# uber/makisu

Measured on AMD Instinct MI355X. Metric: GiB/s hashed (Gear CDC + SHA-256 per chunk), higher is better.
Workload: dtype u32

## Files before the change

### makisu_amd/csrc/gear_cdc.hip

```cpp
#include "mi_common.h"

namespace mi {

typedef u32 u32x4 __attribute__((ext_vector_type(4)));

constexpr int kCopies      = kGearTableCopies;
constexpr int kFastCopies  = 32;
constexpr int kFastWG      = 512;
constexpr int kFastWaves   = kFastWG / 64;

constexpr int kWavesPerWG  = kGearWG / 64;
constexpr int kLaneRun     = kGearTile / 64;
constexpr int kPiece       = 128;
constexpr int kPieceUnits  = kPiece / 16;
constexpr int kBitmapWords = kGearTile / 32;
constexpr int kTableBytes  = 256 * 8 * kCopies;
constexpr int kFastTableBytes = 256 * 8 * kFastCopies;
constexpr int kFastListOff = kFastTableBytes;
constexpr int kFastLdsBytes = kFastListOff + kFastWaves * 64 * 4;
constexpr int kLdsListOff  = kTableBytes + kWavesPerWG * kBitmapWords * 4;
constexpr int kLdsFastOff  = kLdsListOff + kWavesPerWG * 64 * 4;
constexpr int kGearLdsBytes = kLdsFastOff + 16;
constexpr u32 kNoCand = 0xFFFFFFFFu;

__device__ __forceinline__ u32 lane_value(u32 v, int src) { return (u32)__builtin_amdgcn_readlane((int)v, src); }

struct CandPack { u32 a, b; };
__device__ __forceinline__ void cand_push(CandPack& pk, bool& ovf, u32 o) {
    const u32 ca = pk.a >> 30;
    if (ca < 3) { pk.a = ((ca + 1) << 30) | (((pk.a & 0x3FFFFFFFu) << 10) | o); return; }
    const u32 cb = pk.b >> 30;
    if (cb < 3) pk.b = ((cb + 1) << 30) | (((pk.b & 0x3FFFFFFFu) << 10) | o);
    else ovf = true;
}

__device__ __forceinline__ bool cand_compact(CandPack pk, bool ovf, u32 run0, int lane, u32* list) {
    const u32 ca = pk.a >> 30, cb = pk.b >> 30;
    const u32 cnt = ca + cb;
    const u64 b0 = __ballot(cnt & 1u), b1 = __ballot(cnt & 2u), b2 = __ballot(cnt & 4u);
    const u32 total = (u32)__popcll(b0) + 2u * (u32)__popcll(b1) + 4u * (u32)__popcll(b2);
    if (__ballot(ovf) || total > 64u) return false;
    const u64 below = (1ull << lane) - 1ull;
    const u32 first = (u32)__popcll(b0 & below) + 2u * (u32)__popcll(b1 & below) + 4u * (u32)__popcll(b2 & below);
    list[lane] = kNoCand;
#pragma unroll
    for (u32 k = 0; k < 3; ++k)
        if (k < ca) list[first + k] = run0 + ((pk.a >> (10 * (ca - 1 - k))) & 1023u);
    if (cb) {
#pragma unroll
        for (u32 k = 0; k < 3; ++k)
            if (k < cb) list[first + 3 + k] = run0 + ((pk.b >> (10 * (cb - 1 - k))) & 1023u);
    }
    return true;
}

__device__ __forceinline__ int bitmap_find_first(const u64* bm, int lo, int hi, int lane) {
    const int w_lo = lo >> 6, w_hi = hi >> 6;
    for (int w0 = w_lo; w0 <= w_hi; w0 += 64) {
        const int w = w0 + lane;
        u64 v = 0;
        if (w <= w_hi) v = bm[w];
        if (w == w_lo) v &= ~0ull << (lo & 63);
        if (w == w_hi) v &= ~0ull >> (63 - (hi & 63));
        const u64 bal = __ballot(v != 0);
        if (bal) {
            const int src = __ffsll((unsigned long long)bal) - 1;
            const u32 vlo = lane_value((u32)v, src), vhi = lane_value((u32)(v >> 32), src);
            const u64 vv = ((u64)vhi << 32) | vlo;
            return (w0 + src) * 64 + (__ffsll((unsigned long long)vv) - 1);
        }
    }
    return -1;
}

typedef __attribute__((address_space(3))) const u64 lds_cu64;
template <int kC>
__device__ __forceinline__ void roll16(u64& h, const u32x4 v, u32 lane_tab, u32 (&hh)[16]) {
    static_assert(kC == 8 || kC == 16 || kC == 32, "lookup address arithmetic: 64-, 128- or 256-byte entry stride");
    constexpr int kShift = kC == 8 ? 6 : 7;
    constexpr u32 kMask = 0xFFu << kShift;
    const u32 wv[4] = {v.x, v.y, v.z, v.w};
#pragma unroll
    for (int k = 0; k < 16; ++k) {
        const u32 w = wv[k >> 2];
        u32 addr;
        if constexpr (kC == 32) {
            addr = __builtin_amdgcn_perm(w, lane_tab, 0x0C020000u | ((4u + (u32)(k & 3)) << 8));
        } else {
            const int sh = 8 * (k & 3) - kShift;
            const u32 t = sh < 0 ? w << -sh : w >> sh;
            addr = __builtin_amdgcn_bitop3_b32(t, kMask, lane_tab, 0xEA);
        }
        h = (h << 1) + *(lds_cu64*)(size_t)addr;
        hh[k] = (u32)(h >> 32);
    }
}

template <int kC>
__device__ __forceinline__ u32 lds_lane_table(const u64* table, int lane) {
    const u32 base = (u32)(size_t)(__attribute__((address_space(3))) const u64*)table;
    if (base & (u32)(256 * 8 * kC - 1)) __builtin_trap();
    return base | ((u32)(lane % kC) * 8u);
}

__device__ __forceinline__ void load_piece(const u8* p, u32x4 (&d)[kPieceUnits]) {
#pragma unroll
    for (int i = 0; i < kPieceUnits; ++i) d[i] = *(const u32x4*)(p + 16 * i);
}

template <int kC, bool kBitmap>
__device__ __forceinline__ void hash16(u64& h, const u32x4 v, u32 tab, u32 thresh_m1, u32 run0, u32 base,
                                       u32* bitmap, CandPack& pk, bool& ovf) {
    u32 hh[16];
    roll16<kC>(h, v, tab, hh);
    u32 m = 0xFFFFFFFFu;
#pragma unroll
    for (int k = 0; k < 16; k += 2) m = min(m, min(hh[k], hh[k + 1]));
    if (m <= thresh_m1) {
#pragma unroll
        for (int k = 0; k < 16; ++k) {
            if (hh[k] <= thresh_m1) {
                const u32 pos = run0 + base + (u32)k;
                if (kBitmap) atomicOr(&bitmap[pos >> 5], 1u << (pos & 31));
                cand_push(pk, ovf, base + (u32)k);
            }
        }
    }
}

__device__ __forceinline__ void tile_first_loads(const u8* __restrict__ fptr, u64 ts, u32 tlen, int lane,
                                                 u32x4 (&cur)[kPieceUnits], u32x4 (&wq)[4]) {
    const u32 run0 = (u32)lane * kLaneRun;
    if (run0 >= tlen) return;
    const u8* p = fptr + ts + run0;
    load_piece(p, cur);
    if (ts + run0 != 0) {
#pragma unroll
        for (int i = 0; i < 4; ++i) wq[i] = *(const u32x4*)(p - 64 + 16 * i);
    }
}

template <int kC, bool kBitmap>
__device__ __forceinline__ void mark_tile_loaded(const u8* __restrict__ fptr, u64 ts, u32 tlen,
                                                 u32* bitmap, u32 tab, u32 thresh_m1, int lane,
                                                 u32x4 (&cur)[kPieceUnits], const u32x4 (&wq)[4],
                                                 CandPack& pk, bool& ovf) {
    pk.a = pk.b = 0;
    ovf = false;
    const u32 run0 = (u32)lane * kLaneRun;
    if (run0 >= tlen) return;
    const u8* p = fptr + ts + run0;
    const u32 run_len = tlen - run0 < (u32)kLaneRun ? tlen - run0 : (u32)kLaneRun;
    const int n_pieces = (int)((run_len + kPiece - 1) / kPiece);
    u64 h = 0;
    u32 hh[16];
    if (ts + run0 != 0) {
#pragma unroll
        for (int i = 0; i < 4; ++i) roll16<kC>(h, wq[i], tab, hh);
    }
    u32x4 nxt[kPieceUnits];
    for (int pc = 0; pc < n_pieces; ++pc) {
        if (pc + 1 < n_pieces) load_piece(p + (pc + 1) * kPiece, nxt);
#pragma unroll
        for (int g = 0; g < kPieceUnits; ++g)
            hash16<kC, kBitmap>(h, cur[g], tab, thresh_m1, run0, (u32)(pc * kPiece + g * 16), bitmap, pk, ovf);
#pragma unroll
        for (int i = 0; i < kPieceUnits; ++i) cur[i] = nxt[i];
    }
}

template <int kC, bool kBitmap>
__device__ __forceinline__ void mark_tile(const u8* __restrict__ fptr, u64 ts, u32 tlen,
                                          u32* bitmap, u32 tab, u32 thresh_m1, int lane,
                                          CandPack& pk, bool& ovf) {
    if (kBitmap) {
        u32x4* bz = (u32x4*)bitmap;
        const u32x4 z = {0, 0, 0, 0};
#pragma unroll
        for (int i = 0; i < kBitmapWords / 4 / 64; ++i) bz[i * 64 + lane] = z;
    }
    u32x4 cur[kPieceUnits], wq[4];
    tile_first_loads(fptr, ts, tlen, lane, cur, wq);
    mark_tile_loaded<kC, kBitmap>(fptr, ts, tlen, bitmap, tab, thresh_m1, lane, cur, wq, pk, ovf);
}

template <typename Emit>
__device__ __forceinline__ bool select_tile(const u32* bitmap, const u32* list, u64 ts, u32 tlen,
                                            const CdcParams& p, u64& last, int lane, Emit&& emit) {
    const u64 te = ts + tlen;
    const u32 cand = list ? list[lane] : kNoCand;
    for (;;) {
        u64 lo = last + p.min_size;
        if (lo < ts + 1) lo = ts + 1;
        u64 hi = last + p.max_size;
        if (hi > te) hi = te;
        if (lo <= hi) {
            int b;
            if (list) {
                const u32 lo_rel = (u32)(lo - ts - 1), hi_rel = (u32)(hi - ts - 1);
                const u64 bal = __ballot(cand >= lo_rel && cand <= hi_rel);
                b = bal ? (int)lane_value(cand, __ffsll((unsigned long long)bal) - 1) : -1;
            } else {
                b = bitmap_find_first((const u64*)bitmap, (int)(lo - ts - 1), (int)(hi - ts - 1), lane);
            }
            if (b >= 0) {
                last = ts + (u64)b + 1;
                if (emit(last)) return true;
                continue;
            }
        }
        if (last + p.max_size <= te) {
            last += p.max_size;
            if (emit(last)) return true;
            continue;
        }
        break;
    }
    return false;
}

__device__ __forceinline__ bool list_from_bitmap(const u32* bitmap, int lane, u32* list) {
    u32 cnt = 0;
#pragma unroll 4
    for (int w = 0; w < 32; ++w) cnt += (u32)__popc(bitmap[lane * 32 + w]);
    u32 incl = cnt;
#pragma unroll
    for (int d = 1; d < 64; d <<= 1) {
        const u32 y = __shfl_up(incl, d);
        if (lane >= d) incl += y;
    }
    const u32 total = lane_value(incl, 63);
    if (total > 64u) return false;
    list[lane] = kNoCand;
    u32 pos = incl - cnt;
    if (cnt) {
        for (int w = 0; w < 32; ++w) {
            u32 bits = bitmap[lane * 32 + w];
            while (bits) {
                const int b = __ffs(bits) - 1;
                bits &= bits - 1;
                list[pos++] = (u32)lane * kLaneRun + (u32)w * 32u + (u32)b;
            }
        }
    }
    return true;
}

template <int kC, int kWG = kGearWG>
__device__ __forceinline__ void load_table(u64* table, const u64* __restrict__ gear_table, int tid) {
    for (int i = tid; i < 256 * kC; i += kWG) table[i] = gear_table[i / kC];
}

typedef u64 u64x2 __attribute__((ext_vector_type(2)));
__device__ __forceinline__ void load_table_fast(u64* table, const u64* __restrict__ gear_table, int tid) {
    static_assert(kFastWG == 2 * 256 && kFastCopies == 32, "two threads per entry, sixteen copies each");
    const u64 g = gear_table[tid >> 1];
    const u64x2 gg = {g, g};
    u64x2* dst = (u64x2*)(table + (tid >> 1) * kFastCopies + (tid & 1) * (kFastCopies / 2));
#pragma unroll
    for (int i = 0; i < kFastCopies / 4; ++i) dst[i] = gg;
}

__global__ __launch_bounds__(kFastWG)
void gear_cdc_small_fast_kernel(const u8* __restrict__ data, const u64* __restrict__ file_off,
                                const u64* __restrict__ file_size, const u32* __restrict__ seg_file,
                                const u64* __restrict__ seg_slot, u32* __restrict__ ends32,
                                u32* __restrict__ seg_n, const u32* __restrict__ list, u32 n_list,
                                const u64* __restrict__ gear_table, CdcParams p,
                                u32* __restrict__ dense_list, u32* __restrict__ dense_count) {
    extern __shared__ __attribute__((aligned(16))) u8 smem[];
    u64* table = (u64*)smem;
    const int tid = threadIdx.x, lane = tid & 63;
    const int wave = __builtin_amdgcn_readfirstlane(tid >> 6);
    u32* cand_list = (u32*)(smem + kFastListOff) + wave * 64;
    const u32 li = blockIdx.x * kFastWaves + wave;
    const bool have = li < n_list;
    u32 s = 0;
    u64 size = 0, off = 0, slot = 0;
    if (have) {
        s = list[li];
        const u32 f = seg_file[s];
        size = file_size[f];
        off = file_off[f];
        slot = seg_slot[s];
    }
    u32x4 cur[kPieceUnits], wq[4];
    tile_first_loads(data + off, 0, (u32)size, lane, cur, wq);
    load_table_fast(table, gear_table, tid);
    __syncthreads();
    const u32 lane_tab = lds_lane_table<kFastCopies>(table, lane);
    if (!have) return;
    u32* ends = ends32 + slot;
    u64 last = 0;
    u32 n_out = 0;
    if (size) {
        CandPack pk;
        bool ovf;
        mark_tile_loaded<kFastCopies, false>(data + off, 0, (u32)size, nullptr, lane_tab, p.thresh_m1, lane, cur, wq, pk, ovf);
        if (!cand_compact(pk, ovf, (u32)lane * kLaneRun, lane, cand_list)) {
            if (lane == 0) dense_list[atomicAdd(dense_count, 1u)] = s;
            return;
        }
        __builtin_amdgcn_wave_barrier();
        select_tile(nullptr, cand_list, 0, (u32)size, p, last, lane,
                    [&](u64 c) { if (lane == 0) ends[n_out] = (u32)c; ++n_out; return false; });
    }
    if (lane == 0) {
        if (size > last) { ends[n_out] = (u32)size; ++n_out; }
        seg_n[s] = n_out;
    }
}

__global__ __launch_bounds__(kGearWG)
void gear_cdc_small_kernel(const u8* __restrict__ data, const u64* __restrict__ file_off,
                           const u64* __restrict__ file_size, const u32* __restrict__ seg_file,
                           const u64* __restrict__ seg_slot, u32* __restrict__ ends32,
                           u32* __restrict__ seg_n, const u32* __restrict__ list, u32 n_list,
                           const u32* __restrict__ n_list_dev,
                           const u64* __restrict__ gear_table, CdcParams p) {
    extern __shared__ __attribute__((aligned(16))) u8 smem[];
    u64* table = (u64*)smem;
    const int tid = threadIdx.x, lane = tid & 63, wave = tid >> 6;
    if (n_list_dev) {
        n_list = *n_list_dev;
        if (blockIdx.x * kWavesPerWG >= n_list) return;
    }
    u32* bitmap = (u32*)(smem + kTableBytes) + wave * kBitmapWords;
    u32* cand_list = (u32*)(smem + kLdsListOff) + wave * 64;
    load_table<kCopies>(table, gear_table, tid);
    __syncthreads();
    const u32 lane_tab = lds_lane_table<kCopies>(table, lane);
    const u32 li = blockIdx.x * kWavesPerWG + wave;
    if (li >= n_list) return;
    const u32 s = list[li];
    const u32 f = seg_file[s];
    const u64 size = file_size[f];
    u32* ends = ends32 + seg_slot[s];
    u64 last = 0;
    u32 n_out = 0;
    if (size) {
        CandPack pk;
        bool ovf;
        mark_tile<kCopies, true>(data + file_off[f], 0, (u32)size, bitmap, lane_tab, p.thresh_m1, lane,
                                 pk, ovf);
        const bool fast = cand_compact(pk, ovf, (u32)lane * kLaneRun, lane, cand_list);
        __builtin_amdgcn_wave_barrier();
        select_tile(bitmap, fast ? cand_list : nullptr, 0, (u32)size, p, last, lane,
                    [&](u64 c) { if (lane == 0) ends[n_out] = (u32)c; ++n_out; return false; });
    }
    if (lane == 0) {
        if (size > last) { ends[n_out] = (u32)size; ++n_out; }
        seg_n[s] = n_out;
    }
}


__device__ __forceinline__ u64 reselect_group(const u32* lists, const u32* bitmaps, u32 fast_mask,
                                               u64 g0, u64 size, u64 entry, const u32* __restrict__ spec,
                                               u32 spec_n, u64 spec_exit, u32* __restrict__ prefix,
                                               const CdcParams& p, int lane, GroupRec* rec, u32* seg_n_out,
                                               bool open_end) {
    u64 last = entry;
    u32 pcnt = 0, sidx = spec_n;
    u32 sbase = 0;
    u32 sreg = lane < (int)spec_n ? spec[lane] : kNoCand;
    bool synced = false;
    auto emit = [&](u64 c) -> bool {
        const u32 rel = (u32)(c - g0);
        for (;;) {
            const u64 bal = __ballot(sreg >= rel);
            if (bal) {
                const int i = __ffsll((unsigned long long)bal) - 1;
                if (lane_value(sreg, i) == rel && sbase + (u32)i < spec_n) { sidx = sbase + (u32)i; synced = true; }
                break;
            }
            if (sbase + 64u >= spec_n) break;
            sbase += 64u;
            sreg = sbase + (u32)lane < spec_n ? spec[sbase + lane] : kNoCand;
        }
        if (synced) return true;
        if (lane == 0) prefix[pcnt] = rel;
        ++pcnt;
        return false;
    };
    for (int t = 0; t < kWavesPerWG && !synced; ++t) {
        const u64 tts = g0 + (u64)t * kGearTile;
        if (tts >= size) break;
        const u32 tlen = (u32)((size - tts < (u64)kGearTile) ? (size - tts) : (u64)kGearTile);
        select_tile(bitmaps + t * kBitmapWords, (fast_mask >> t) & 1u ? lists + t * 64 : nullptr, tts, tlen,
                    p, last, lane, emit);
    }
    if (!synced && !open_end && g0 + kGroupBytes >= size && size > last) {
        if (!emit(size)) last = size;
    }
    const u64 exit = synced ? spec_exit : last;
    if (lane == 0) {
        rec->entry = entry;
        rec->pcnt = pcnt;
        rec->sidx = sidx;
        rec->final_exit = exit;
        rec->flags = (rec->flags & kGroupDense) | kGroupValid;
        *seg_n_out = pcnt + (spec_n - sidx);
    }
    return exit;
}

__global__ __launch_bounds__(kFastWG)
void gear_tile_mark_kernel(const u8* __restrict__ data, const u64* __restrict__ file_off,
                           const u64* __restrict__ file_size, const u32* __restrict__ group_file,
                           const u32* __restrict__ group_index, u32 n_groups,
                           u32* __restrict__ tile_lists, u32* __restrict__ tile_fast,
                           const u64* __restrict__ gear_table, CdcParams p) {
    extern __shared__ __attribute__((aligned(16))) u8 smem[];
    u64* table = (u64*)smem;
    const int tid = threadIdx.x, lane = tid & 63;
    const int wave = __builtin_amdgcn_readfirstlane(tid >> 6);
    u32* cl = (u32*)(smem + kFastListOff) + wave * 64;
    const u64 gw = (u64)blockIdx.x * kFastWaves + (u64)wave;
    const u32 g = (u32)(gw / kWavesPerWG);
    const bool have = g < n_groups;
    const int tw = (int)(gw % kWavesPerWG);
    const u64 t = (u64)g * kWavesPerWG + tw;
    u64 size = 0, off = 0, ts = 0;
    if (have) {
        const u32 f = group_file[g];
        size = file_size[f];
        off = file_off[f];
        ts = (u64)group_index[g] * kGroupBytes + (u64)tw * kGearTile;
    }
    const u32 tlen = ts >= size ? 0u : (u32)((size - ts < (u64)kGearTile) ? (size - ts) : (u64)kGearTile);
    u32x4 cur[kPieceUnits], wq[4];
    tile_first_loads(data + off, ts, tlen, lane, cur, wq);
    load_table_fast(table, gear_table, tid);
    __syncthreads();
    const u32 lane_tab = lds_lane_table<kFastCopies>(table, lane);
    if (!have) return;
    bool fast = true;
    if (tlen) {
        CandPack pk;
        bool ovf;
        mark_tile_loaded<kFastCopies, false>(data + off, ts, tlen, nullptr, lane_tab, p.thresh_m1, lane, cur, wq, pk, ovf);
        fast = cand_compact(pk, ovf, (u32)lane * kLaneRun, lane, cl);
        __builtin_amdgcn_wave_barrier();
        tile_lists[t * 64 + lane] = fast ? cl[lane] : kNoCand;
    }
    if (lane == 0) tile_fast[t] = fast ? 1u : 0u;
}

__global__ __launch_bounds__(kGearWG)
void gear_group_spec_kernel(const u64* __restrict__ file_size, const u64* __restrict__ file_seg0,
                            const u64* __restrict__ seg_slot, u32* __restrict__ ends32,
                            u32* __restrict__ seg_n, const u32* __restrict__ group_file,
                            const u32* __restrict__ group_index, u32 n_groups,
                            GroupRec* __restrict__ recs, const u32* __restrict__ tile_lists,
                            const u32* __restrict__ tile_fast, const u32* __restrict__ file_flags,
                            CdcParams p) {
    __shared__ u32 lists[kWavesPerWG][kWavesPerWG * 64];
    const int lane = threadIdx.x & 63, wave = threadIdx.x >> 6;
    const u32 g = blockIdx.x * kWavesPerWG + wave;
    if (g >= n_groups) return;
    const u32 f = group_file[g], gi = group_index[g];
    const u64 size = file_size[f];
    const bool open_end = file_flags && (file_flags[f] & kFileOpenEnd);
    const u64 g0 = (u64)gi * kGroupBytes;
    const u64 s = file_seg0[f] + gi;
    u32 fast_mask = 0;
#pragma unroll
    for (int t = 0; t < kWavesPerWG; ++t) {
        lists[wave][t * 64 + lane] = tile_lists[((u64)g * kWavesPerWG + t) * 64 + lane];
        fast_mask |= (tile_fast[(u64)g * kWavesPerWG + t] ? 1u : 0u) << t;
    }
    __builtin_amdgcn_wave_barrier();
    GroupRec r;
    r.pcnt = 0;
    r.sidx = 0;
    r.entry = gi == 0 ? 0ull : ~0ull;
    if (fast_mask != (1u << kWavesPerWG) - 1u) {
        r.spec_exit = r.final_exit = ~0ull;
        r.spec_n = 0;
        r.flags = kGroupDense;
        if (lane == 0) { recs[g] = r; seg_n[s] = 0; }
        return;
    }
    u32* spec = ends32 + seg_slot[s];
    u64 last = g0;
    u32 n_out = 0;
    for (int t = 0; t < kWavesPerWG; ++t) {
        const u64 tts = g0 + (u64)t * kGearTile;
        if (tts >= size) break;
        const u32 tlen = (u32)((size - tts < (u64)kGearTile) ? (size - tts) : (u64)kGearTile);
        select_tile(nullptr, lists[wave] + t * 64, tts, tlen, p, last, lane,
                    [&](u64 c) { if (lane == 0) spec[n_out] = (u32)(c - g0); ++n_out; return false; });
    }
    if (lane == 0) {
        if (!open_end && g0 + kGroupBytes >= size && size > last) {
            spec[n_out] = (u32)(size - g0); ++n_out; last = size;
        }
        r.spec_exit = last;
        r.spec_n = n_out;
        r.final_exit = last;
        r.flags = 0;
        if (gi == 0) { r.flags |= kGroupValid; seg_n[s] = n_out; }
        recs[g] = r;
    }
}

__global__ __launch_bounds__(kGearWG)
void gear_group_validate_kernel(const u64* __restrict__ file_size, const u64* __restrict__ file_seg0,
                                const u64* __restrict__ seg_slot, u32* __restrict__ ends32,
                                u32* __restrict__ seg_n, const u32* __restrict__ group_file,
                                const u32* __restrict__ group_index, u32 n_groups,
                                GroupRec* __restrict__ recs, const u32* __restrict__ tile_lists,
                                const u32* __restrict__ file_flags, u32 region, CdcParams p) {
    __shared__ u32 lists[kWavesPerWG][kWavesPerWG * 64];
    const int lane = threadIdx.x & 63, wave = threadIdx.x >> 6;
    const u32 g = blockIdx.x * kWavesPerWG + wave;
    if (g >= n_groups) return;
    const u32 gi = group_index[g];
    if (gi == 0) return;
    GroupRec* rec = recs + g;
    if ((rec->flags | recs[g - 1].flags) & kGroupDense) return;
    const u32 f = group_file[g];
    const u64 s = file_seg0[f] + gi;
#pragma unroll
    for (int t = 0; t < kWavesPerWG; ++t)
        lists[wave][t * 64 + lane] = tile_lists[((u64)g * kWavesPerWG + t) * 64 + lane];
    __builtin_amdgcn_wave_barrier();
    u32* spec = ends32 + seg_slot[s];
    (void)reselect_group(lists[wave], nullptr, (1u << kWavesPerWG) - 1u, (u64)gi * kGroupBytes, file_size[f],
                         recs[g - 1].spec_exit, spec, rec->spec_n, rec->spec_exit, spec + region, p, lane,
                         rec, seg_n + s, file_flags && (file_flags[f] & kFileOpenEnd));
}

__global__ __launch_bounds__(kGearWG)
void gear_file_fix_kernel(const u8* __restrict__ data, const u64* __restrict__ file_off,
                          const u64* __restrict__ file_size, const u64* __restrict__ file_seg0,
                          const u64* __restrict__ seg_slot, u32* __restrict__ ends32,
                          u32* __restrict__ seg_n, const u32* __restrict__ large_list,
                          const u32* __restrict__ large_group0, GroupRec* __restrict__ recs,
                          const u32* __restrict__ tile_lists, const u32* __restrict__ file_flags,
                          u32 region, const u64* __restrict__ gear_table, CdcParams p) {
    extern __shared__ __attribute__((aligned(16))) u8 smem[];
    u64* table = (u64*)smem;
    const int tid = threadIdx.x, lane = tid & 63, wave = tid >> 6;
    u32* bitmaps = (u32*)(smem + kTableBytes);
    u32* cand_lists = (u32*)(smem + kLdsListOff);
    volatile u32* fast_flags = (volatile u32*)(smem + kLdsFastOff);
    volatile u32* s_next = (volatile u32*)(smem + kGearLdsBytes);
    volatile u64* s_entry = (volatile u64*)(smem + kGearLdsBytes + 8);
    const u32 f = large_list[blockIdx.x];
    const u64 size = file_size[f];
    const u8* fptr = data + file_off[f];
    const u32 gb = large_group0[blockIdx.x];
    const bool open_end = file_flags && (file_flags[f] & kFileOpenEnd);
    const u32 ng = (u32)((size + kGroupBytes - 1) / kGroupBytes);
    u32 gi = 0;
    u64 prev_exit = 0;
    bool have_table = false;
    u32 lane_tab = 0;
    for (;;) {
        if (wave == 0) {
            u32 redo = 0xFFFFFFFFu, dense = 0;
            while (gi < ng) {
                bool bad[4];
                u64 ex[4];
#pragma unroll
                for (int k = 0; k < 4; ++k) {
                    const u32 my = gi + (u32)(k * 64 + lane);
                    bad[k] = false;
                    ex[k] = 0;
                    if (my < ng) {
                        const GroupRec r = recs[gb + my];
                        const u64 pe = my == gi ? prev_exit : recs[gb + my - 1].final_exit;
                        ex[k] = r.final_exit;
                        bad[k] = !(r.flags & kGroupValid) || r.entry != pe;
                    }
                }
                bool stop = false;
#pragma unroll
                for (int k = 0; k < 4 && !stop; ++k) {
                    if (gi >= ng) break;
                    const u64 bal = __ballot(bad[k]);
                    if (!bal) {
                        const u32 n = ng - gi < 64u ? ng - gi : 64u;
                        const u32 lo = lane_value((u32)ex[k], (int)n - 1), hi = lane_value((u32)(ex[k] >> 32), (int)n - 1);
                        prev_exit = ((u64)hi << 32) | lo;
                        gi += n;
                        continue;
                    }
                    const int j = __ffsll((unsigned long long)bal) - 1;
                    if (j > 0) {
                        const u32 lo = lane_value((u32)ex[k], j - 1), hi = lane_value((u32)(ex[k] >> 32), j - 1);
                        prev_exit = ((u64)hi << 32) | lo;
                    }
                    gi += (u32)j;
                    redo = gi;
                    dense = recs[gb + gi].flags & kGroupDense;
                    stop = true;
                }
                if (stop) break;
            }
            if (lane == 0) { s_next[0] = redo; s_next[1] = dense; *s_entry = prev_exit; }
        }
        __syncthreads();
        const u32 redo = s_next[0];
        if (redo == 0xFFFFFFFFu) break;
        if (!have_table) {
            load_table<kCopies>(table, gear_table, tid);
            __syncthreads();
            lane_tab = lds_lane_table<kCopies>(table, lane);
            have_table = true;
        }
        const u32 g = gb + redo;
        const u64 g0 = (u64)redo * kGroupBytes;
        if (s_next[1]) {
            const u64 ts = g0 + (u64)wave * kGearTile;
            if (lane == 0) fast_flags[wave] = 1u;
            if (ts < size) {
                const u32 tlen = (u32)((size - ts < (u64)kGearTile) ? (size - ts) : (u64)kGearTile);
                CandPack pk;
                bool ovf;
                u32* bm = bitmaps + wave * kBitmapWords;
                u32* cl = cand_lists + wave * 64;
                mark_tile<kCopies, true>(fptr, ts, tlen, bm, lane_tab, p.thresh_m1, lane, pk, ovf);
                bool fast = cand_compact(pk, ovf, (u32)lane * kLaneRun, lane, cl);
                if (!fast) {
                    __builtin_amdgcn_wave_barrier();
                    fast = list_from_bitmap(bm, lane, cl);
                }
                if (lane == 0) fast_flags[wave] = fast ? 1u : 0u;
            }
        } else {
            cand_lists[wave * 64 + lane] = tile_lists[((u64)g * kWavesPerWG + wave) * 64 + lane];
            if (lane == 0) fast_flags[wave] = 1u;
        }
        __syncthreads();
        if (wave == 0) {
            u32 fast_mask = 0;
            for (int t = 0; t < kWavesPerWG; ++t) fast_mask |= (fast_flags[t] ? 1u : 0u) << t;
            const u64 s = file_seg0[f] + redo;
            u32* spec = ends32 + seg_slot[s];
            GroupRec* rec = recs + g;
            const u64 entry = *s_entry;
            prev_exit = reselect_group(cand_lists, bitmaps, fast_mask, g0, size, entry, spec, rec->spec_n,
                                       rec->spec_exit, spec + region, p, lane, rec, seg_n + s, open_end);
            gi = redo + 1;
        }
        __syncthreads();
    }
}

u64 gear_large_groups(u64 size) { return (size + kGroupBytes - 1) / kGroupBytes; }
u64 gear_group_region(u32 min_size) { return kGroupBytes / min_size + 2; }
size_t gear_group_rec_bytes() { return sizeof(GroupRec); }

static void gear_lds_attributes() {
    static thread_local int done_for = -1;
    int dev = 0;
    (void)hipGetDevice(&dev);
    if (done_for == dev) return;
    (void)hipFuncSetAttribute((const void*)gear_cdc_small_kernel,
                              hipFuncAttributeMaxDynamicSharedMemorySize, kGearLdsBytes);
    (void)hipFuncSetAttribute((const void*)gear_cdc_small_fast_kernel,
                              hipFuncAttributeMaxDynamicSharedMemorySize, kFastLdsBytes);
    (void)hipFuncSetAttribute((const void*)gear_tile_mark_kernel,
                              hipFuncAttributeMaxDynamicSharedMemorySize, kFastLdsBytes);
    (void)hipFuncSetAttribute((const void*)gear_file_fix_kernel,
                              hipFuncAttributeMaxDynamicSharedMemorySize, kGearLdsBytes + 16);
    done_for = dev;
}

void launch_gear_cdc(const GearLaunch& a, CdcParams p, int n_cu, hipStream_t s) {
    (void)n_cu;
    gear_lds_attributes();
    if (a.n_small) {
        const dim3 grid((a.n_small + kWavesPerWG - 1) / kWavesPerWG);
        const dim3 fast_grid((a.n_small + kFastWaves - 1) / kFastWaves);
        const bool try_fast = a.dense_list && p.thresh_m1 <= 0x003FFFFFu;
        if (try_fast) {
            (void)hipMemsetAsync(a.dense_count, 0, 4, s);
            hipLaunchKernelGGL(gear_cdc_small_fast_kernel, fast_grid, dim3(kFastWG), kFastLdsBytes, s, a.data,
                               a.file_off, a.file_size, a.seg_file, a.seg_slot, a.ends32, a.seg_n, a.small_list,
                               a.n_small, a.gear_table, p, a.dense_list, a.dense_count);
            hipLaunchKernelGGL(gear_cdc_small_kernel, grid, dim3(kGearWG), kGearLdsBytes, s, a.data, a.file_off,
                               a.file_size, a.seg_file, a.seg_slot, a.ends32, a.seg_n, a.dense_list, 0u,
                               (const u32*)a.dense_count, a.gear_table, p);
        } else {
            hipLaunchKernelGGL(gear_cdc_small_kernel, grid, dim3(kGearWG), kGearLdsBytes, s, a.data, a.file_off,
                               a.file_size, a.seg_file, a.seg_slot, a.ends32, a.seg_n, a.small_list, a.n_small,
                               (const u32*)nullptr, a.gear_table, p);
        }
    }
    if (a.n_groups) {
        const u32 region = (u32)gear_group_region(p.min_size);
        GroupRec* recs = (GroupRec*)a.group_recs;
        const u64 n_tiles = (u64)a.n_groups * kWavesPerWG;
        hipLaunchKernelGGL(gear_tile_mark_kernel, dim3((u32)((n_tiles + kFastWaves - 1) / kFastWaves)), dim3(kFastWG), kFastLdsBytes, s, a.data,
                           a.file_off, a.file_size, a.group_file, a.group_index, a.n_groups, a.tile_lists,
                           a.tile_fast, a.gear_table, p);
        const dim3 per_group((a.n_groups + kWavesPerWG - 1) / kWavesPerWG);
        hipLaunchKernelGGL(gear_group_spec_kernel, per_group, dim3(kGearWG), 0, s, a.file_size, a.file_seg0,
                           a.seg_slot, a.ends32, a.seg_n, a.group_file, a.group_index, a.n_groups, recs,
                           a.tile_lists, a.tile_fast, a.file_flags, p);
        if (a.n_groups > a.n_large)
            hipLaunchKernelGGL(gear_group_validate_kernel, per_group, dim3(kGearWG), 0, s, a.file_size,
                               a.file_seg0, a.seg_slot, a.ends32, a.seg_n, a.group_file, a.group_index,
                               a.n_groups, recs, a.tile_lists, a.file_flags, region, p);
        hipLaunchKernelGGL(gear_file_fix_kernel, dim3(a.n_large), dim3(kGearWG), kGearLdsBytes + 16, s,
                           a.data, a.file_off, a.file_size, a.file_seg0, a.seg_slot, a.ends32, a.seg_n,
                           a.large_list, a.large_group0, recs, a.tile_lists, a.file_flags, region,
                           a.gear_table, p);
    }
}

__global__ __launch_bounds__(64)
void part_apply_kernel(const u32* __restrict__ part_group0, const u32* __restrict__ part_halo,
                       const u64* __restrict__ part_entry, u32 n_parts, GroupRec* __restrict__ recs) {
    const u32 i = blockIdx.x * blockDim.x + threadIdx.x;
    if (i >= n_parts || part_halo[i] == 0 || part_entry[i] == ~0ull) return;
    recs[part_group0[i] + part_halo[i] - 1].final_exit = part_entry[i];
}

__global__ __launch_bounds__(64)
void part_halo_clear_kernel(const u32* __restrict__ part_file, const u32* __restrict__ part_halo,
                            u32 n_parts, const u64* __restrict__ file_seg0, u32* __restrict__ seg_n) {
    const u32 i = blockIdx.x;
    if (i >= n_parts) return;
    const u64 s0 = file_seg0[part_file[i]];
    for (u32 g = threadIdx.x; g < part_halo[i]; g += blockDim.x) seg_n[s0 + g] = 0;
}

void launch_gear_parts(const GearLaunch& a, const u32* d_part_file, const u32* d_part_group0,
                       const u32* d_part_halo, const u64* d_part_entry, u32 n_parts, bool refix,
                       CdcParams p, hipStream_t s) {
    if (n_parts == 0) return;
    GroupRec* recs = (GroupRec*)a.group_recs;
    if (refix) {
        const u32 region = (u32)gear_group_region(p.min_size);
        hipLaunchKernelGGL(part_apply_kernel, dim3((n_parts + 63) / 64), dim3(64), 0, s, d_part_group0,
                           d_part_halo, d_part_entry, n_parts, recs);
        hipLaunchKernelGGL(gear_file_fix_kernel, dim3(n_parts), dim3(kGearWG), kGearLdsBytes + 16, s,
                           a.data, a.file_off, a.file_size, a.file_seg0, a.seg_slot, a.ends32, a.seg_n,
                           d_part_file, d_part_group0, recs, a.tile_lists, a.file_flags, region,
                           a.gear_table, p);
    }
    hipLaunchKernelGGL(part_halo_clear_kernel, dim3(n_parts), dim3(64), 0, s, d_part_file, d_part_halo,
                       n_parts, a.file_seg0, a.seg_n);
}

}
```

Before: 1086.

## Reuse neighbour lane's rolling hash instead of reloading a 64-byte warmup window

In the non-bitmap Gear CDC path, each lane no longer loads and rolls the 64 bytes before its run to warm up the hash. Lanes now hash their run from a zero state and skip candidates in the first 64 bytes. They then take the previous lane's final 64-bit hash via shfl_up and re-hash their first 64 bytes to recover those candidates, which are packed into a new small head list merged during compaction. This removes a redundant per-lane global load of the overlap window, at the cost of extra registers, a cross-lane shuffle, and tighter overflow limits on the head list (at most 4 head candidates, 6 total per lane).

```diff
diff --git a/makisu_amd/csrc/gear_cdc.hip b/makisu_amd/csrc/gear_cdc.hip
--- a/makisu_amd/csrc/gear_cdc.hip
+++ b/makisu_amd/csrc/gear_cdc.hip
@@ -34,15 +34,30 @@
     else ovf = true;
 }
 
-__device__ __forceinline__ bool cand_compact(CandPack pk, bool ovf, u32 run0, int lane, u32* list) {
+__device__ __forceinline__ void head_push(u32& hp, bool& ovf, u32 o) {
+    const u32 c = hp >> 29;
+    if (c < 4) hp = ((c + 1) << 29) | (((hp & 0x3FFFFu) << 6) | o);
+    else ovf = true;
+}
+
+template <bool kHead = false>
+__device__ __forceinline__ bool cand_compact(CandPack pk, bool ovf, u32 run0, int lane, u32* list, u32 hp = 0) {
     const u32 ca = pk.a >> 30, cb = pk.b >> 30;
-    const u32 cnt = ca + cb;
+    const u32 ch = kHead ? hp >> 29 : 0u;
+    const u32 cnt = ca + cb + ch;
+    if (kHead) ovf = ovf || cnt > 6u;
     const u64 b0 = __ballot(cnt & 1u), b1 = __ballot(cnt & 2u), b2 = __ballot(cnt & 4u);
     const u32 total = (u32)__popcll(b0) + 2u * (u32)__popcll(b1) + 4u * (u32)__popcll(b2);
     if (__ballot(ovf) || total > 64u) return false;
     const u64 below = (1ull << lane) - 1ull;
-    const u32 first = (u32)__popcll(b0 & below) + 2u * (u32)__popcll(b1 & below) + 4u * (u32)__popcll(b2 & below);
+    u32 first = (u32)__popcll(b0 & below) + 2u * (u32)__popcll(b1 & below) + 4u * (u32)__popcll(b2 & below);
     list[lane] = kNoCand;
+    if (kHead && ch) {
+#pragma unroll
+        for (u32 k = 0; k < 4; ++k)
+            if (k < ch) list[first + k] = run0 + ((hp >> (6 * (ch - 1 - k))) & 63u);
+        first += ch;
+    }
 #pragma unroll
     for (u32 k = 0; k < 3; ++k)
         if (k < ca) list[first + k] = run0 + ((pk.a >> (10 * (ca - 1 - k))) & 1023u);
@@ -110,7 +125,7 @@
 
 template <int kC, bool kBitmap>
 __device__ __forceinline__ void hash16(u64& h, const u32x4 v, u32 tab, u32 thresh_m1, u32 run0, u32 base,
-                                       u32* bitmap, CandPack& pk, bool& ovf) {
+                                       u32* bitmap, CandPack& pk, bool& ovf, u32 skip = 0) {
     u32 hh[16];
     roll16<kC>(h, v, tab, hh);
     u32 m = 0xFFFFFFFFu;
@@ -119,7 +134,7 @@
     if (m <= thresh_m1) {
 #pragma unroll
         for (int k = 0; k < 16; ++k) {
-            if (hh[k] <= thresh_m1) {
+            if (hh[k] <= thresh_m1 && base >= skip) {
                 const u32 pos = run0 + base + (u32)k;
                 if (kBitmap) atomicOr(&bitmap[pos >> 5], 1u << (pos & 31));
                 cand_push(pk, ovf, base + (u32)k);
@@ -128,13 +143,28 @@
     }
 }
 
+template <int kC>
+__device__ __forceinline__ void head16(u64& h, const u32x4 v, u32 tab, u32 thresh_m1, u32 base, u32& hp, bool& ovf) {
+    u32 hh[16];
+    roll16<kC>(h, v, tab, hh);
+    u32 m = 0xFFFFFFFFu;
+#pragma unroll
+    for (int k = 0; k < 16; k += 2) m = min(m, min(hh[k], hh[k + 1]));
+    if (m <= thresh_m1) {
+#pragma unroll
+        for (int k = 0; k < 16; ++k)
+            if (hh[k] <= thresh_m1) head_push(hp, ovf, base + (u32)k);
+    }
+}
+
+template <bool kBitmap>
 __device__ __forceinline__ void tile_first_loads(const u8* __restrict__ fptr, u64 ts, u32 tlen, int lane,
                                                  u32x4 (&cur)[kPieceUnits], u32x4 (&wq)[4]) {
     const u32 run0 = (u32)lane * kLaneRun;
     if (run0 >= tlen) return;
     const u8* p = fptr + ts + run0;
     load_piece(p, cur);
-    if (ts + run0 != 0) {
+    if (kBitmap ? ts + run0 != 0 : (ts != 0 && run0 == 0)) {
 #pragma unroll
         for (int i = 0; i < 4; ++i) wq[i] = *(const u32x4*)(p - 64 + 16 * i);
     }
@@ -144,10 +174,43 @@
 __device__ __forceinline__ void mark_tile_loaded(const u8* __restrict__ fptr, u64 ts, u32 tlen,
                                                  u32* bitmap, u32 tab, u32 thresh_m1, int lane,
                                                  u32x4 (&cur)[kPieceUnits], const u32x4 (&wq)[4],
-                                                 CandPack& pk, bool& ovf) {
+                                                 CandPack& pk, bool& ovf, u32& hp) {
     pk.a = pk.b = 0;
+    hp = 0;
     ovf = false;
     const u32 run0 = (u32)lane * kLaneRun;
+    if constexpr (!kBitmap) {
+        const bool active = run0 < tlen;
+        const u8* p = fptr + ts + run0;
+        const u32 run_len = !active ? 0u : tlen - run0 < (u32)kLaneRun ? tlen - run0 : (u32)kLaneRun;
+        const int n_pieces = (int)((run_len + kPiece - 1) / kPiece);
+        u64 h = 0;
+        if (ts != 0 && run0 == 0 && active) {
+            u32 hw[16];
+#pragma unroll
+            for (int i = 0; i < 4; ++i) roll16<kC>(h, wq[i], tab, hw);
+        }
+        const u32 skip = lane == 0 ? 0u : 64u;
+        u32x4 head[4];
+#pragma unroll
+        for (int i = 0; i < 4; ++i) head[i] = cur[i];
+        u32x4 nxt[kPieceUnits];
+        for (int pc = 0; pc < n_pieces; ++pc) {
+            if (pc + 1 < n_pieces) load_piece(p + (pc + 1) * kPiece, nxt);
+#pragma unroll
+            for (int g = 0; g < kPieceUnits; ++g)
+                hash16<kC, false>(h, cur[g], tab, thresh_m1, run0, (u32)(pc * kPiece + g * 16), bitmap, pk, ovf, skip);
+#pragma unroll
+            for (int i = 0; i < kPieceUnits; ++i) cur[i] = nxt[i];
+        }
+        const u32 lo = __shfl_up((u32)h, 1), hi = __shfl_up((u32)(h >> 32), 1);
+        if (active && lane != 0) {
+            u64 hl = ((u64)hi << 32) | lo;
+#pragma unroll
+            for (int i = 0; i < 4; ++i) head16<kC>(hl, head[i], tab, thresh_m1, (u32)(16 * i), hp, ovf);
+        }
+        return;
+    }
     if (run0 >= tlen) return;
     const u8* p = fptr + ts + run0;
     const u32 run_len = tlen - run0 < (u32)kLaneRun ? tlen - run0 : (u32)kLaneRun;
@@ -180,8 +243,9 @@
         for (int i = 0; i < kBitmapWords / 4 / 64; ++i) bz[i * 64 + lane] = z;
     }
     u32x4 cur[kPieceUnits], wq[4];
-    tile_first_loads(fptr, ts, tlen, lane, cur, wq);
-    mark_tile_loaded<kC, kBitmap>(fptr, ts, tlen, bitmap, tab, thresh_m1, lane, cur, wq, pk, ovf);
+    u32 hp;
+    tile_first_loads<kBitmap>(fptr, ts, tlen, lane, cur, wq);
+    mark_tile_loaded<kC, kBitmap>(fptr, ts, tlen, bitmap, tab, thresh_m1, lane, cur, wq, pk, ovf, hp);
 }
 
 template <typename Emit>
@@ -285,7 +349,7 @@
         slot = seg_slot[s];
     }
     u32x4 cur[kPieceUnits], wq[4];
-    tile_first_loads(data + off, 0, (u32)size, lane, cur, wq);
+    tile_first_loads<false>(data + off, 0, (u32)size, lane, cur, wq);
     load_table_fast(table, gear_table, tid);
     __syncthreads();
     const u32 lane_tab = lds_lane_table<kFastCopies>(table, lane);
@@ -296,8 +360,9 @@
     if (size) {
         CandPack pk;
         bool ovf;
-        mark_tile_loaded<kFastCopies, false>(data + off, 0, (u32)size, nullptr, lane_tab, p.thresh_m1, lane, cur, wq, pk, ovf);
-        if (!cand_compact(pk, ovf, (u32)lane * kLaneRun, lane, cand_list)) {
+        u32 hp;
+        mark_tile_loaded<kFastCopies, false>(data + off, 0, (u32)size, nullptr, lane_tab, p.thresh_m1, lane, cur, wq, pk, ovf, hp);
+        if (!cand_compact<true>(pk, ovf, (u32)lane * kLaneRun, lane, cand_list, hp)) {
             if (lane == 0) dense_list[atomicAdd(dense_count, 1u)] = s;
             return;
         }
@@ -430,7 +495,7 @@
     }
     const u32 tlen = ts >= size ? 0u : (u32)((size - ts < (u64)kGearTile) ? (size - ts) : (u64)kGearTile);
     u32x4 cur[kPieceUnits], wq[4];
-    tile_first_loads(data + off, ts, tlen, lane, cur, wq);
+    tile_first_loads<false>(data + off, ts, tlen, lane, cur, wq);
     load_table_fast(table, gear_table, tid);
     __syncthreads();
     const u32 lane_tab = lds_lane_table<kFastCopies>(table, lane);
@@ -439,8 +504,9 @@
     if (tlen) {
         CandPack pk;
         bool ovf;
-        mark_tile_loaded<kFastCopies, false>(data + off, ts, tlen, nullptr, lane_tab, p.thresh_m1, lane, cur, wq, pk, ovf);
-        fast = cand_compact(pk, ovf, (u32)lane * kLaneRun, lane, cl);
+        u32 hp;
+        mark_tile_loaded<kFastCopies, false>(data + off, ts, tlen, nullptr, lane_tab, p.thresh_m1, lane, cur, wq, pk, ovf, hp);
+        fast = cand_compact<true>(pk, ovf, (u32)lane * kLaneRun, lane, cl, hp);
         __builtin_amdgcn_wave_barrier();
         tile_lists[t * 64 + lane] = fast ? cl[lane] : kNoCand;
     }
```

New measurement: 1101 (median of 6 runs). 1.4% higher.
